# consensus-shipyard/ipc-filecoin-proofs

Hardware: NVIDIA H100
Metric: receipts/sec scanned (higher is better)
Workload: dtype u8

## Files before the change

ipc_filecoin_proofs_b200/csrc/engine.cuh:

```cuda
#pragma once
#include <array>
#include <memory>
#include <mutex>
#include <string>
#include <vector>

#include "common.cuh"
#include "store.cuh"
#include "rawcid.cuh"

namespace ipcfp {

struct NumaPrefer {
    bool on = false;
    int old_mode = 0;
    unsigned long old_mask[16] = {};
    explicit NumaPrefer(int device);
    ~NumaPrefer();
};

struct PinnedPool {
    struct Buf { void* p; size_t cap; };
    std::mutex mu;
    std::vector<Buf> free_list;
// ... 7 lines not shown
    size_t cap = 0;
    PinnedArray() {}
    PinnedArray(std::shared_ptr<PinnedPool> pl, size_t bytes) : pool(std::move(pl)) { p = pool->take(bytes ? bytes : 16, &cap); }
    PinnedArray(const PinnedArray&) = delete;
    PinnedArray& operator=(const PinnedArray&) = delete;
    PinnedArray(PinnedArray&& o) noexcept : pool(std::move(o.pool)), p(o.p), cap(o.cap) { o.p = nullptr; }
    PinnedArray& operator=(PinnedArray&& o) noexcept { release(); pool = std::move(o.pool); p = o.p; cap = o.cap; o.p = nullptr; return *this; }
    ~PinnedArray() { release(); }
    void release() { if (p && pool) pool->give(p, cap); p = nullptr; }
    template <class T> T* as() const { return (T*)p; }
};

struct Store {
    int device = 0;
    cudaStream_t stream = nullptr, stream2 = nullptr;
    uint64_t n = 0, blob_size = 0;
    DevBuf<uint8_t> arena;
    DevBuf<uint64_t> offsets;
    DevBuf<uint32_t> lengths;
    DevBuf<Digest> digests;
    DevBuf<uint8_t> cls;
    DevBuf<uint64_t> table;
    DevBuf<BlockRec> recs;
    DevBuf<uint32_t> rank_of, block_at_rank;
    StoreView view{};
    DevBuf<StoreView> view_dev;
    std::vector<std::array<uint8_t, 6>> class_prefix;
    std::vector<uint32_t> class_rank;
    uint64_t first_bad = UINT64_MAX;
    std::shared_ptr<PinnedPool> pool;
// ... 181 lines not shown
```

ipc_filecoin_proofs_b200/csrc/events.cu:

```cuda
#include <algorithm>
#include <cstdlib>
#include <cstring>

#include <chrono>
#include "engine.cuh"
#include "hashes.cuh"
#include "ipld.cuh"
#include "prims.cuh"
#include "walk.cuh"
#include "events_items.cuh"
#include "pass1_stage.cuh"
#include "rawcid.cuh"

namespace ipcfp {


__global__ void k_check_exec(const uint32_t* __restrict__ match_rel, uint64_t n_match, uint64_t lo, const unsigned long long* __restrict__ n_exec,
                             unsigned long long* err) {
    uint64_t t = (uint64_t)blockIdx.x * blockDim.x + threadIdx.x;
    if (t >= n_match) return;
    const uint64_t i = lo + match_rel[t];
    if (i >= *n_exec) report_error(err, ST_PASS2, i, 0 , 0);
}
__global__ void __launch_bounds__(128) k_pass2(Pass2Args a) {
    uint64_t t = (uint64_t)blockIdx.x * blockDim.x + threadIdx.x;
    if (a.per_warp) { if (threadIdx.x & 31) return; t >>= 5; }
    if (t >= a.n_match) return;
    pass2_item(a, t);
}

#define IPCFP_MAX_PARENTS 64
struct SetupArgs {
    StoreView store;
    uint32_t n_parents;
    const uint8_t* parent_cids;
    const uint8_t* txmeta_cids;
    const uint8_t* child_cid;
    const uint8_t* receipts_root;
    uint32_t skip_tx;
    uint32_t skip_receipts;
    uint32_t* wbits;
    unsigned long long* err;
    unsigned long long* txerr;
    uint32_t* receipts_root_blk;
    uint32_t* f_blk; uint32_t* f_meta; uint64_t* f_base;
    unsigned long long* f_count;
    uint32_t* amt_height;
    uint64_t* amt_count;
    uint32_t* missing_base;
    const uint8_t* sig;
    uint32_t sig_len;
    Matcher* matcher;
};

__global__ void __launch_bounds__(256) k_setup(SetupArgs a) {
    const StoreView& s = a.store;
    const uint32_t t = threadIdx.x, P = a.n_parents;
    if (t >= 128 && !a.skip_tx) {
        for (uint32_t i = t - 128; i < 2 * P + 2; i += 128) {
            const uint8_t* cid = i < P ? a.parent_cids + 38 * i : (i == P ? a.child_cid : (i == P + 1 ? a.receipts_root : a.txmeta_cids + 38 * (i - P - 2)));
            int32_t b = store_lookup(s, cid);
            if (b < 0) *a.missing_base = 1; else witness_mark(s, a.wbits, (uint32_t)b);
        }
    }
    if (t == 96) {
        Digest d;
        keccak256(a.sig, a.sig_len, d);
        a.matcher->t0[0] = d.w[0]; a.matcher->t0[1] = d.w[1]; a.matcher->t0[2] = d.w[2]; a.matcher->t0[3] = d.w[3];
    }
    if (t >= 32 && t < 96) for (uint32_t b = t - 32; b < P; b += 64) {
        for (uint32_t k = 0; k < 2; k++) { a.f_meta[2 * b + k] = AMT_SENTINEL; a.f_blk[2 * b + k] = 0; a.f_base[2 * b + k] = 0; a.amt_height[2 * b + k] = 0; a.amt_count[2 * b + k] = 0; }
        int32_t tb = store_lookup(s, a.txmeta_cids + 38 * b);
        if (tb < 0) { report_tx_error(a.txerr, 3 * b, 0, 31, DC_MISSING, 0); continue; }
        if (!a.skip_tx) witness_mark(s, a.wbits, (uint32_t)tb);
        uint32_t len;
        const uint8_t* p = store_block(s, (uint32_t)tb, len);
        Rd r(p, len);
        rd_array_exact(r, 2);
        uint32_t c0 = rd_cid(r), c1 = rd_cid(r);
        rd_end(r);
        if (r.err) { report_tx_error(a.txerr, 3 * b, 0, 31, DC_DECODE, r.err); continue; }
        for (uint32_t k = 0; k < 2; k++) {
            int32_t rb = store_lookup(s, p + (k ? c1 : c0));
            if (rb < 0) { report_tx_error(a.txerr, 3 * b + 1 + k, 0, 31, DC_MISSING, 0); break; }
            if (!a.skip_tx) witness_mark(s, a.wbits, (uint32_t)rb);
            uint32_t rl;
            const uint8_t* rp = store_block(s, (uint32_t)rb, rl);
            Rd rr(rp, rl);
            uint32_t bw, h;
            uint64_t cnt;
            amt_root_begin(rr, 0, bw, h, cnt);
            if (rr.err) { report_tx_error(a.txerr, 3 * b + 1 + k, 0, 31, DC_DECODE, rr.err); break; }
            const uint32_t amt = 2 * b + k;
            a.f_blk[amt] = (uint32_t)rb;
            a.f_meta[amt] = make_meta(amt, 1, h);
            a.f_base[amt] = 0;
            a.amt_height[amt] = h;
            a.amt_count[amt] = cnt;
        }
    }
    if (t != 0) return;
    *a.f_count = 2 * P;
    if (a.skip_receipts) return;
    int32_t rb = store_lookup(s, a.receipts_root);
    if (rb < 0) { report_error(a.err, ST_RECEIPTS_ROOT, 0, DC_MISSING, 0); return; }
    witness_mark(s, a.wbits, (uint32_t)rb);
    *a.receipts_root_blk = (uint32_t)rb;
    uint32_t len;
    const uint8_t* p = store_block(s, (uint32_t)rb, len);
    Rd r(p, len);
    uint32_t bw, h;
    uint64_t cnt;
    amt_root_begin(r, 0, bw, h, cnt);
    AmtNodeHdr hd;
    amt_node_begin(r, 3, hd);
    uint32_t nv = rd_array(r);
    for (uint32_t v = 0; v < nv && !r.err; v++) parse_receipt(r);
    amt_node_finish(r, hd, nv, h);
    if (r.err) report_error(a.err, ST_RECEIPTS_ROOT, 0, DC_DECODE, r.err);
}

__global__ void __launch_bounds__(128) k_amt_count(StoreView store, Frontier in, const unsigned long long* in_count, uint32_t round, uint32_t last_round,
                                                   uint32_t cap, uint32_t* counts, const uint64_t* rlo, const uint64_t* rhi) {
    uint64_t t = (uint64_t)blockIdx.x * blockDim.x + threadIdx.x;
    uint64_t cnt = *in_count;
    if (cnt > cap) cnt = cap;
    if (t >= cnt) { counts[t] = 0; return; }
    counts[t] = amt_item_count(store, in.blk[t], in.meta[t], in.base[t], round, last_round, rlo, rhi);
}
__global__ void __launch_bounds__(128) k_amt_expand(ExpandArgs a, const uint32_t* counts, unsigned long long* out_count, const unsigned long long* total) {
    const uint64_t g = (uint64_t)blockIdx.x * blockDim.x + threadIdx.x;
    const uint64_t t = g >> 3;
    const uint32_t j = (uint32_t)g & 7;
    uint64_t cnt = *a.in_count;
// ... 40 lines not shown
        ExpandArgs a = a0;
        a.in = cur; a.out = nxt; a.round = round; a.out_off = scan_tmp;
        for (uint32_t it = t >> 3; it < cnt; it += TOP_CAP / 8) amt_item_expand(a, it, t & 7, cur.blk[it], cur.meta[it], cur.base[it], s_cnt[it]);
        __syncthreads();
        if (t == 0) {
            unsigned long long n = s_total;
            if (round < a0.last_round && n > a0.cap) { report_tx_error(a0.err, IPCFP_TX_EIDX_NONE, 0, 0, DC_UNSUPPORTED, 1); n = a0.cap; }
            *count_io = n;
        }
        __threadfence();
        __syncthreads();
        Frontier tmp = cur; cur = nxt; nxt = tmp;
    }
}

__global__ void __launch_bounds__(1024) k_amt_dense(DenseArgs a, uint32_t first_round, uint32_t n_rounds) {
    for (uint32_t rr = 0; rr < n_rounds; rr++) {
        const uint32_t round = first_round + rr;
        if (*(volatile uint32_t*)a.fail) return;
        const Frontier in = (round & 1) ? a.pong : a.ping, out = (round & 1) ? a.ping : a.pong;
        const uint64_t n8 = (uint64_t)a.ftot[round] * 8;
        for (uint64_t g = (uint64_t)blockIdx.x * blockDim.x + threadIdx.x; g < n8; g += (uint64_t)gridDim.x * blockDim.x)
            amt_item_dense(a, in, out, round, (uint32_t)(g >> 3), (uint32_t)g & 7);
        if (n_rounds > 1) { __threadfence(); __syncthreads(); }
    }
}

__global__ void k_dedup_insert(const RawCid* __restrict__ raw, uint64_t n, unsigned long long* table, uint64_t mask) {
    uint64_t i = (uint64_t)blockIdx.x * blockDim.x + threadIdx.x;
    if (i >= n) return;
    RawCid c = raw[i];
    uint64_t h = rawcid_hash(c);
    uint32_t fp = (uint32_t)(h >> 32) | 1u;
    unsigned long long mine = ((unsigned long long)fp << 32) | (unsigned long long)(i + 1);
    uint64_t slot = h & mask;
    for (;;) {
        unsigned long long e = table[slot];
        if (e == 0) { e = atomicCAS(&table[slot], 0ull, mine); if (e == 0) return; }
        if ((uint32_t)(e >> 32) == fp && rawcid_eq(raw[(uint32_t)e - 1], c)) { atomicMin(&table[slot], mine); return; }
        slot = (slot + 1) & mask;
// ... 163 lines not shown
    {
        uint8_t* hs = s->stage.as<uint8_t>();
        memset(hs, 0, small_bytes);
        memcpy(hs, &mh, sizeof(Matcher));
        memcpy(hs + 1024, spec->event_signature, siglen);
        uint8_t* hc = hs + 1024 + sig_cap;
        memcpy(hc, td.parent_cids.data(), td.parent_cids.size()); hc += td.parent_cids.size();
        memcpy(hc, td.txmeta_cids.data(), td.txmeta_cids.size()); hc += td.txmeta_cids.size();
        memcpy(hc, td.child_cid, 38); hc += 38;
        memcpy(hc, td.receipts_root, 38);
        IPCFP_CUDA(cudaMemcpyAsync(small.p, hs, small_bytes, cudaMemcpyHostToDevice, st));
    }

    AsyncBuf<uint32_t> wbits((nblk + 31) / 32 + 8, st);
    wbits.zero();
    const uint32_t namt_max = 2 * td.n_parents;
    const uint64_t cap = 4 * nblk + 1024;
    AsyncBuf<uint32_t> fA_blk(cap, st), fA_meta(cap, st), fB_blk(cap, st), fB_meta(cap, st);
    AsyncBuf<uint64_t> fA_base(cap, st), fB_base(cap, st);
    AsyncBuf<uint32_t> misc(64 + 2 * IPCFP_MAX_PARENTS, st);
    AsyncBuf<uint64_t> amt_count(2 * IPCFP_MAX_PARENTS, st);
    misc.zero();
    SetupArgs sa;
    sa.store = s->view; sa.n_parents = td.n_parents;
    sa.parent_cids = d_cids; sa.txmeta_cids = d_cids + 38ull * td.n_parents;
    sa.child_cid = d_cids + 76ull * td.n_parents; sa.receipts_root = sa.child_cid + 38;
    sa.skip_tx = skip_tx; sa.skip_receipts = exo ? 1 : 0; sa.wbits = wbits.p; sa.err = dw; sa.txerr = dw + 15;
    sa.receipts_root_blk = misc.p; sa.missing_base = misc.p + 1; sa.amt_height = misc.p + 64;
    sa.f_blk = fA_blk.p; sa.f_meta = fA_meta.p; sa.f_base = fA_base.p; sa.f_count = dw + 1;
    sa.amt_count = amt_count.p;
    sa.sig = d_sig; sa.sig_len = (uint32_t)siglen; sa.matcher = d_matcher;
    k_setup<<<1, 256, 0, st>>>(sa); IPCFP_LAUNCH_CHECK();
    IPCFP_CUDA(cudaMemcpyAsync(hw + 400, d_matcher, 32, cudaMemcpyDeviceToHost, st));
    IPCFP_CUDA(cudaMemcpyAsync(hw + 24, misc.p, (64 + 2 * IPCFP_MAX_PARENTS) * 4, cudaMemcpyDeviceToHost, st));
    IPCFP_CUDA(cudaMemcpyAsync(hw + 128, amt_count.p, 2 * IPCFP_MAX_PARENTS * 8, cudaMemcpyDeviceToHost, st));
    IPCFP_CUDA(cudaMemcpyAsync(hw, dw, 16 * 8, cudaMemcpyDeviceToHost, st));
    IPCFP_CUDA(cudaStreamSynchronize(st));
    const bool early_fault = hw[0] != IPCFP_NO_ERROR || hw[15] != IPCFP_NO_ERROR;
    memcpy(mh.t0, hw + 400, 32);
    const uint32_t* misc_h = (const uint32_t*)(hw + 24);
    const uint32_t receipts_root_blk = misc_h[0];
    const bool missing_base = misc_h[1] != 0;
    uint32_t namt = (uint32_t)hw[1];
    uint32_t last_round = 0;
    for (uint32_t k = 0; k < namt && k < namt_max; k++) last_round = std::max(last_round, misc_h[64 + k]);

    IPCFP_CUDA(cudaEventRecord(s->ev[1], st));
    std::vector<uint64_t> h_rng(4 * IPCFP_MAX_PARENTS, 0);
    const uint64_t nraw_total = shard_amt_ranges(namt, (const uint64_t*)(hw + 128), sharded, lo, hi, td.n_receipts, h_rng.data(),
                                                 h_rng.data() + 2 * IPCFP_MAX_PARENTS);
    AsyncBuf<uint32_t> counts(cap + 1024, st);
    AsyncBuf<uint64_t> out_off(cap + 1024, st), scratch(scan_scratch_elems(std::max<uint64_t>(cap, N) + 64) + 64, st);
    unsigned long long *ccount = dw + 1, *ncount = dw + 2, *total_dev = dw + 13;
    const uint32_t frontier_cap = (uint32_t)std::min<uint64_t>(cap, 0xffffffffull);
    AsyncBuf<RawCid> exec_raw;
    uint64_t raw_cap = 0;

    const bool force_general = getenv("IPCFP_BFS_GENERAL") != nullptr;
    DensePlan plan;
    if (namt > 0 && namt <= namt_max && !force_general && !early_fault)
        plan = make_dense_plan(namt, misc_h + 64, (const uint64_t*)(hw + 128), h_rng.data(), h_rng.data() + 2 * IPCFP_MAX_PARENTS, frontier_cap, 8ull * cap,
                               STAGE_TABLES);
    AsyncBuf<uint8_t> d_tables;
    AsyncBuf<uint64_t> d_foff;
    AsyncBuf<uint32_t> d_flen;
    auto run_dense = [&]() {
        const size_t nb_amt = plan.per_amt.size() * 8, nb_fofs = plan.fofs.size() * 4, nb_ftot = plan.ftot.size() * 4;
        uint8_t* ht = s->stage.as<uint8_t>() + tables_off;
        memcpy(ht, plan.per_amt.data(), nb_amt);
        memcpy(ht + nb_amt, plan.fofs.data(), nb_fofs);
        memcpy(ht + nb_amt + nb_fofs, plan.ftot.data(), nb_ftot);
        d_tables.alloc(nb_amt + nb_fofs + nb_ftot + 64, st);
        IPCFP_CUDA(cudaMemcpyAsync(d_tables.p, ht, nb_amt + nb_fofs + nb_ftot, cudaMemcpyHostToDevice, st));
        raw_cap = plan.nraw;
        exec_raw.alloc(raw_cap + 64, st);
        exec_raw.zero();
        DenseArgs da;
        da.store = s->view;
        da.ping = Frontier{fA_blk.p, fA_meta.p, fA_base.p}; da.pong = Frontier{fB_blk.p, fB_meta.p, fB_base.p};
        da.vals = exec_raw.p;
        const uint64_t* pa = (const uint64_t*)d_tables.p;
        da.vbase = pa; da.cnt = pa + namt; da.lo = pa + 2ull * namt; da.hi = pa + 3ull * namt;
        da.fofs = (const uint32_t*)(d_tables.p + nb_amt); da.ftot = (const uint32_t*)(d_tables.p + nb_amt + nb_fofs);
        da.namt = namt; da.record = skip_tx ? 0 : 1; da.wbits = wbits.p; da.fail = (uint32_t*)(dw + 14);
        uint64_t fmax = 1;
        for (uint32_t r = 0; r < plan.rounds; r++) fmax = std::max<uint64_t>(fmax, plan.ftot[r]);
        d_foff.alloc(2 * fmax + 8, st); d_flen.alloc(2 * fmax + 8, st);
        da.f_off[0] = d_foff.p; da.f_off[1] = d_foff.p + fmax; da.f_len[0] = d_flen.p; da.f_len[1] = d_flen.p + fmax;
        uint32_t top = 0;
        while (top < plan.rounds && plan.ftot[top] <= 1024) top++;
        if (top) { k_amt_dense<<<1, 1024, 0, st>>>(da, 0, top); IPCFP_LAUNCH_CHECK(); }
        for (uint32_t r = top; r < plan.rounds; r++) {
            k_amt_dense<<<div_up((uint64_t)plan.ftot[r] * 8, 256), 256, 0, st>>>(da, r, 1); IPCFP_LAUNCH_CHECK();
        }
    };

    AsyncBuf<uint64_t> d_rng;
    auto run_general = [&]() {
        d_rng.alloc(4 * IPCFP_MAX_PARENTS, st);
        IPCFP_CUDA(cudaMemcpyAsync(d_rng.p, h_rng.data(), h_rng.size() * 8, cudaMemcpyHostToDevice, st));
        IPCFP_CUDA(cudaStreamSynchronize(st));
        Frontier fcur{fA_blk.p, fA_meta.p, fA_base.p}, fnxt{fB_blk.p, fB_meta.p, fB_base.p};
        ccount = dw + 1; ncount = dw + 2;
        ExpandArgs ea;
        ea.store = s->view; ea.last_round = last_round; ea.record = skip_tx ? 0 : 1; ea.wbits = wbits.p; ea.err = dw + 15;
        ea.vals = nullptr; ea.cap = frontier_cap;
        ea.rlo = d_rng.p; ea.rhi = d_rng.p + 2 * IPCFP_MAX_PARENTS;
        auto bound_of = [&](uint32_t round) { uint64_t b = namt; for (uint32_t k = 0; k < round && b <= cap; k++) b *= 8; return std::min<uint64_t>(b, cap); };
        auto alloc_vals = [&]() {
            raw_cap = std::min<uint64_t>(bound_of(last_round) * 8, 8 * cap);
// ... 13 lines not shown
            round = top_rounds;
        }
        for (; round <= last_round; round++) {
            uint64_t items = bound_of(round);
            if (round == last_round) alloc_vals();
            unsigned grid = div_up(std::max<uint64_t>(items, 1), 128);
            k_amt_count<<<grid, 128, 0, st>>>(s->view, fcur, ccount, round, last_round, ea.cap, counts.p, ea.rlo, ea.rhi); IPCFP_LAUNCH_CHECK();
            exclusive_scan_u32(counts.p, out_off.p, (uint64_t)grid * 128, (uint64_t*)total_dev, scratch.p, st);
            ExpandArgs a = ea;
            a.in = fcur; a.in_count = ccount; a.out = fnxt; a.round = round; a.out_off = out_off.p;
            k_amt_expand<<<div_up(std::max<uint64_t>(items, 1) * 8, 128), 128, 0, st>>>(a, counts.p, ncount, total_dev); IPCFP_LAUNCH_CHECK();
            std::swap(fcur, fnxt);
            std::swap(ccount, ncount);
        }
    };
    bool dense_used = plan.ok;
    if (dense_used) run_dense(); else run_general();
    IPCFP_CUDA(cudaEventRecord(s->ev[9], st));
    bool xch_early = false;
    if (xch) {
        xch->agree_early(plan.ok && !early_fault, plan.ok ? plan.nraw : 0, nraw_total);
        xch_early = xch->all_early;
        if (xch_early) xch->start_exchange(exec_raw.p, s->ev[9]);
    }
    WitnessBuilder wbuild(s);
    wbuild.by_ref = (flags & IPCFP_WITNESS_BY_REFERENCE) != 0;
    if (!exo) wbuild.snapshot(wbits.p);
    publish_words(s, 0, 18);
    IPCFP_CUDA(cudaStreamSynchronize(st));
    if (dense_used && hw[14] != 0) {
        dense_used = false;
        k_setup<<<1, 256, 0, st>>>(sa); IPCFP_LAUNCH_CHECK();
        run_general();
        IPCFP_CUDA(cudaEventRecord(s->ev[9], st));
        if (!exo) wbuild.snapshot(wbits.p);
        publish_words(s, 0, 18);
        IPCFP_CUDA(cudaStreamSynchronize(st));
    }
    const uint32_t ccount_idx = (uint32_t)(ccount - dw);
    note_errors(hw);
    if (!dense_used && hw[ccount_idx] > raw_cap) {
        if (!xch) throw Error(IPCFP_ERR_UNSUPPORTED, "unsupported input (message list longer than the walk's capacity)");
        pend_tx = std::min<uint64_t>(pend_tx, tx_err_key(IPCFP_TX_EIDX_NONE, 0, 0, DC_UNSUPPORTED, 1));
    }
    uint64_t nraw = dense_used ? plan.nraw : std::min<uint64_t>(hw[ccount_idx], raw_cap);
    bool xch_stale = xch_early && (!dense_used || nraw != plan.nraw);
    if (xch && !xch_early && (pend_tx != IPCFP_NO_ERROR || pend_err != IPCFP_NO_ERROR)) {
        xch->agree_slices(pend_tx, pend_err, 0);
        throw_global(xch->g_tx, xch->g_err, false);
    }
    if (!exo) wbuild.start_copy(hw[8], hw[9], hw[16], hw[17]);
    if (xch && !xch_early) {
        xch->agree_slices(IPCFP_NO_ERROR, IPCFP_NO_ERROR, nraw);
        if (!xch->peers_ok) { IPCFP_CUDA(cudaStreamSynchronize(st)); throw_global(xch->g_tx, xch->g_err, false); }
        xch->start_exchange(exec_raw.p, s->ev[9]);
    }
    AsyncBuf<uint32_t> exec_idx(nraw + 32, st), keep_bits((nraw + 31) / 32 + 8, st);
    unsigned long long* n_exec_dev = dw + 3;
    if (sharded) IPCFP_CUDA(cudaMemsetAsync(n_exec_dev, 0, 8, st));
    else if (nraw) {
// ... 34 lines not shown
    bitmap_to_indices(match_bits.p, (N + 31) / 32 * 32, match_rel.p, (uint64_t*)n_match_dev, wp3.p, scratch.p, st);
    exclusive_scan_u32(cnt.p, pbase.p, N, (uint64_t*)(dw + 7), scratch.p, st);
    exclusive_scan_u32(nby.p, bbase.p, N, (uint64_t*)(dw + 12), scratch.p, st);
    publish_words(s, 0, 16);
    IPCFP_CUDA(cudaStreamSynchronize(st));
    note_errors(hw);
    uint64_t n_exec = hw[3];
    const uint64_t M = hw[6];
    const uint64_t pass1_nodes = hw[4], pass1_bytes = hw[5];
    uint64_t n_proofs = hw[7], n_bytes = hw[12];

    std::unique_ptr<EventResultBox> box(new EventResultBox());
    memset(&box->r, 0, sizeof box->r);
    AsyncBuf<ipcfp_event_proof> d_proofs(n_proofs + 1, st);
    AsyncBuf<uint8_t> d_blob(n_bytes + 16, st);
    uint32_t* any_skip_dev = misc.p + 2;
    if (M) {
        Pass2Args p2;
        p2.store = s->view; p2.store_dev = s->view_dev.p; p2.m_dev = d_matcher; p2.m = mh; p2.events_roots = td.events_roots.p; p2.lo = lo; p2.match_rel = match_rel.p; p2.n_match = M;
        p2.receipts_root_blk = receipts_root_blk; p2.exec_cids = exec_raw.p; p2.exec_idx = exec_idx.p; p2.n_exec = n_exec_dev;
        p2.wbits = wbits.p; p2.err = dw; p2.cnt = cnt.p; p2.proof_base = pbase.p; p2.byte_base = bbase.p;
        p2.proofs = d_proofs.p; p2.blob = d_blob.p; p2.any_skip = any_skip_dev; p2.resolve_msg = sharded ? 0 : 1;
        p2.per_warp = (M <= 16384 && !getenv("IPCFP_PASS2_PER_THREAD")) ? 1 : 0;
        k_pass2<<<div_up(p2.per_warp ? M * 32 : M, 128), 128, 0, st>>>(p2); IPCFP_LAUNCH_CHECK();
    }
    if (xch) {
        cudaStream_t sx = xch->stream();
        xch->positions_for(sx, match_rel.p, M, n_exec_dev);
        IPCFP_CUDA(cudaMemsetAsync(dw + 19, 0xff, 8, sx));
        if (M) { k_check_exec<<<div_up(M, 128), 128, 0, sx>>>(match_rel.p, M, lo, n_exec_dev, dw + 19); IPCFP_LAUNCH_CHECK(); }
        publish_words_on(s, sx, dw + 19, 19, 1);
    }
    wbuild.finish_enqueue(wbits.p);
    publish_words(s, 0, 20);
    publish_words_from(s, misc.p, 20, 2);
    IPCFP_CUDA(cudaStreamSynchronize(st));
    note_errors(hw);
    if (!xch && missing_base && !skip_tx) throw Error(IPCFP_ERR_MISSING_BLOCK, "missing block (base witness CID not in the store)");
    const uint64_t mB = hw[10];
    const bool any_skip = ((const uint32_t*)(hw + 20))[2] != 0;
    IPCFP_CUDA(cudaEventRecord(s->ev[4], st));

    box->matching = PinnedArray(s->pool, (M + 1) * 8);
    box->proofs = PinnedArray(s->pool, (n_proofs + 1) * sizeof(ipcfp_event_proof));
    box->blob = PinnedArray(s->pool, n_bytes + 16);
    PinnedArray rel(s->pool, (M + 1) * 4);
    if (M) IPCFP_CUDA(cudaMemcpyAsync(rel.p, match_rel.p, M * 4, cudaMemcpyDeviceToHost, st));
    if (n_proofs && !xch) IPCFP_CUDA(cudaMemcpyAsync(box->proofs.p, d_proofs.p, n_proofs * sizeof(ipcfp_event_proof), cudaMemcpyDeviceToHost, st));
    if (n_bytes) IPCFP_CUDA(cudaMemcpyAsync(box->blob.p, d_blob.p, n_bytes, cudaMemcpyDeviceToHost, st));

// ... 137 lines not shown
```

ipc_filecoin_proofs_b200/csrc/walk.cuh:

```cuda
#pragma once
#include <algorithm>
#include <vector>

#include "ipld.cuh"
#include "rawcid.cuh"

namespace ipcfp {

__device__ __forceinline__ uint32_t make_meta(uint32_t amt, uint32_t is_root, uint32_t level) { return (amt << 16) | (is_root << 8) | level; }

#define AMT_SENTINEL 0xffffffffu

struct Frontier { uint32_t* blk; uint32_t* meta; uint64_t* base; };

__device__ __forceinline__ uint32_t slot_mask(uint64_t base, uint32_t level, uint64_t rlo, uint64_t rhi) {
    uint64_t sub = pow_sat(3, level);
    uint32_t m = 0;
#pragma unroll
    for (uint32_t sl = 0; sl < 8; sl++) {
        uint64_t off = sub == ~0ull ? (sl ? ~0ull : 0) : sub * sl;
        uint64_t cb = base + off < base ? ~0ull : base + off;
        uint64_t ce = cb + sub < cb ? ~0ull : cb + sub;
        if (cb < rhi && ce > rlo) m |= 1u << sl;
    }
// ... 79 lines not shown
                } else {
                    const uint8_t* src = p + vals_off + 43 * j + 5;
                    RawCid c;
                    c.w[4] = load_u64_any(src) & 0xffffffffffffull;
                    Digest dg = load_digest(src + 6);
                    c.w[0] = dg.w[0]; c.w[1] = dg.w[1]; c.w[2] = dg.w[2]; c.w[3] = dg.w[3];
                    a.vals[d] = c;
                }
            }
        }
    }
    if (a.round < a.last_round) for (uint32_t k = produced + j; k < expect; k += 8) if (o + k < a.cap) a.out.meta[o + k] = AMT_SENTINEL;
    if (a.round == a.last_round) for (uint32_t k = produced + j; k < expect; k += 8) { RawCid z{}; a.vals[o + k] = z; }
}

struct DenseArgs {
    StoreView store;
    Frontier ping, pong;
    RawCid* vals;
    const uint32_t* fofs;
    const uint32_t* ftot;
    const uint64_t* vbase;
    const uint64_t* cnt;
    const uint64_t* lo;
    const uint64_t* hi;
    uint32_t namt, record;
    uint32_t* wbits;
    uint32_t* fail;
    uint64_t* f_off[2];
    uint32_t* f_len[2];
};
__device__ __forceinline__ void amt_item_dense(const DenseArgs& a, const Frontier& in, const Frontier& out, uint32_t round, uint32_t it, uint32_t j) {
    const uint32_t meta = in.meta[it];
    const uint64_t base = in.base[it];
    const uint32_t level = meta & 0xff, is_root = (meta >> 8) & 1, amt = meta >> 16;
    uint32_t len;
    const uint8_t* p;
    if (round == 0) p = store_block(a.store, in.blk[it], len);
    else { const uint32_t par = round & 1; len = a.f_len[par][it]; p = a.store.blob + a.f_off[par][it]; }
    uint32_t q0 = 0;
    if (is_root) {
        Rd r(p, len);
        uint32_t bw, h; uint64_t c;
        amt_root_begin(r, 0, bw, h, c);
        if (r.err) { *a.fail = 1; return; }
// ... 50 lines not shown
        glo = n_receipts ? (uint64_t)((__uint128_t)nraw_total * lo / n_receipts) : 0;
        ghi = n_receipts ? (uint64_t)((__uint128_t)nraw_total * hi / n_receipts) : 0;
    }
    for (uint32_t k = 0; k < namt; k++) {
        uint64_t A0 = rawbase[k], A1 = rawbase[k + 1];
        uint64_t l = glo > A0 ? glo - A0 : 0, h = ghi > A0 ? ghi - A0 : 0;
        if (!sharded) { l = 0; h = UINT64_MAX; }
        else if (glo >= A1 && !(A1 == A0 && glo == A0)) { l = h = 0; }
        else if (ghi >= A1) h = UINT64_MAX;
        if (h < l) h = l;
        range_lo[k] = l; range_hi[k] = h;
    }
    return nraw_total;
}

struct DensePlan {
    bool ok = false;
    uint32_t rounds = 0;
    uint64_t nraw = 0;
    std::vector<uint32_t> fofs, ftot;
    std::vector<uint64_t> per_amt;
};
inline DensePlan make_dense_plan(uint32_t namt, const uint32_t* heights, const uint64_t* cnts, const uint64_t* range_lo, const uint64_t* range_hi,
                                 uint64_t frontier_cap, uint64_t max_raw, size_t max_table_bytes) {
    DensePlan plan;
    bool ok = namt > 0;
    uint32_t last_round = 0;
    for (uint32_t k = 0; ok && k < namt; k++) {
        ok = heights[k] <= 20 && cnts[k] <= (1ull << 40) && cnts[k] <= (1ull << (3 * (heights[k] + 1)));
        last_round = std::max(last_round, heights[k]);
    }
    if (ok) {
        plan.rounds = last_round + 1;
        plan.fofs.assign((size_t)plan.rounds * namt, 0);
        plan.ftot.assign(plan.rounds, 0);
        plan.per_amt.assign(4ull * namt, 0);
        uint64_t vb = 0;
        for (uint32_t k = 0; k < namt; k++) {
            const uint64_t c = cnts[k];
            const uint64_t l = std::min(range_lo[k], c), h = std::max(l, std::min(range_hi[k], c));
            if (l == h && l > 0) ok = false;
            plan.per_amt[k] = vb; plan.per_amt[namt + k] = c; plan.per_amt[2ull * namt + k] = l; plan.per_amt[3ull * namt + k] = h;
            vb += h - l;
        }
        plan.nraw = vb;
        for (uint32_t r = 0; ok && r < plan.rounds; r++) {
            uint64_t run = 0;
            for (uint32_t k = 0; k < namt; k++) {
                plan.fofs[(size_t)r * namt + k] = (uint32_t)run;
                const uint32_t hk = heights[k];
                if (r > hk) continue;
                const uint64_t l = plan.per_amt[2ull * namt + k], h = plan.per_amt[3ull * namt + k];
                const uint32_t sh = 3 * (hk - r + 1);
                uint64_t nodes = r == 0 ? 1 : (l < h ? (sh >= 64 ? 1 : ((h - 1) >> sh) - (l >> sh) + 1) : 0);
                run += nodes;
                if (run > frontier_cap) { ok = false; break; }
            }
            plan.ftot[r] = (uint32_t)run;
        }
        const size_t tbytes = plan.fofs.size() * 4 + plan.ftot.size() * 4 + plan.per_amt.size() * 8 + 64;
        if (plan.nraw > max_raw || tbytes > max_table_bytes) ok = false;
    }
    plan.ok = ok;
    return plan;
}

}
```

Measured before the change: 549.9 million.

## Build dense AMT walk plan on device and run walk as cooperative kernel

Moves the dense-walk planning from the host onto the device, inside the setup kernel, for the non-sharded case. This removes the mid-pipeline stream synchronize and device-to-host copy of the prologue that the host planner needed. The per-round walk launches are replaced by one cooperative kernel that uses grid.sync between levels, followed by a separate leaf kernel. The cost is a conservatively sized raw buffer (max_raw_dev), the exec_raw zeroing is dropped on the device-planned path, and the walk now depends on cooperative launch and grid occupancy.

```diff
diff --git a/ipc_filecoin_proofs_b200/csrc/engine.cuh b/ipc_filecoin_proofs_b200/csrc/engine.cuh
--- a/ipc_filecoin_proofs_b200/csrc/engine.cuh
+++ b/ipc_filecoin_proofs_b200/csrc/engine.cuh
@@ -45,6 +45,7 @@
 struct Store {
     int device = 0;
     cudaStream_t stream = nullptr, stream2 = nullptr;
+    unsigned walk_grid = 0;
     uint64_t n = 0, blob_size = 0;
     DevBuf<uint8_t> arena;
     DevBuf<uint64_t> offsets;
diff --git a/ipc_filecoin_proofs_b200/csrc/events.cu b/ipc_filecoin_proofs_b200/csrc/events.cu
--- a/ipc_filecoin_proofs_b200/csrc/events.cu
+++ b/ipc_filecoin_proofs_b200/csrc/events.cu
@@ -3,6 +3,8 @@
 #include <cstring>
 
 #include <chrono>
+#include <cstddef>
+#include <cooperative_groups.h>
 #include "engine.cuh"
 #include "hashes.cuh"
 #include "ipld.cuh"
@@ -13,6 +15,7 @@
 #include "rawcid.cuh"
 
 namespace ipcfp {
+namespace cg = cooperative_groups;
 
 
 __global__ void k_check_exec(const uint32_t* __restrict__ match_rel, uint64_t n_match, uint64_t lo, const unsigned long long* __restrict__ n_exec,
@@ -30,6 +33,16 @@
 }
 
 #define IPCFP_MAX_PARENTS 64
+static_assert(2 * IPCFP_MAX_PARENTS <= DENSE_MAX_AMTS, "the dense plan's tables hold every message AMT");
+struct Prologue {
+    uint32_t misc[64 + 2 * IPCFP_MAX_PARENTS];
+    uint64_t amt_count[2 * IPCFP_MAX_PARENTS];
+    uint64_t t0[4];
+    DenseTables plan;
+};
+#define PRO_HOST_WORD 24
+static constexpr uint32_t PRO_HEAD_WORDS = (uint32_t)((offsetof(Prologue, plan) + offsetof(DenseTables, per_amt)) / 8);
+static_assert(PRO_HOST_WORD + PRO_HEAD_WORDS <= 300, "the prologue's head must not reach the sharded protocol's host words");
 struct SetupArgs {
     StoreView store;
     uint32_t n_parents;
@@ -42,34 +55,55 @@
     uint32_t* wbits;
     unsigned long long* err;
     unsigned long long* txerr;
-    uint32_t* receipts_root_blk;
+    Prologue* pro;
     uint32_t* f_blk; uint32_t* f_meta; uint64_t* f_base;
     unsigned long long* f_count;
-    uint32_t* amt_height;
-    uint64_t* amt_count;
-    uint32_t* missing_base;
     const uint8_t* sig;
     uint32_t sig_len;
     Matcher* matcher;
+    uint32_t plan_dense;
+    uint64_t frontier_cap, max_raw;
 };
+
+__device__ __forceinline__ void setup_receipts_root(const SetupArgs& a) {
+    const StoreView& s = a.store;
+    int32_t rb = store_lookup(s, a.receipts_root);
+    if (rb < 0) { report_error(a.err, ST_RECEIPTS_ROOT, 0, DC_MISSING, 0); return; }
+    witness_mark(s, a.wbits, (uint32_t)rb);
+    a.pro->misc[0] = (uint32_t)rb;
+    uint32_t len;
+    const uint8_t* p = store_block(s, (uint32_t)rb, len);
+    Rd r(p, len);
+    uint32_t bw, h;
+    uint64_t cnt;
+    amt_root_begin(r, 0, bw, h, cnt);
+    AmtNodeHdr hd;
+    amt_node_begin(r, 3, hd);
+    uint32_t nv = rd_array(r);
+    for (uint32_t v = 0; v < nv && !r.err; v++) parse_receipt(r);
+    amt_node_finish(r, hd, nv, h);
+    if (r.err) report_error(a.err, ST_RECEIPTS_ROOT, 0, DC_DECODE, r.err);
+}
 
 __global__ void __launch_bounds__(256) k_setup(SetupArgs a) {
     const StoreView& s = a.store;
     const uint32_t t = threadIdx.x, P = a.n_parents;
+    uint32_t* const amt_height = a.pro->misc + 64;
+    uint64_t* const amt_count = a.pro->amt_count;
     if (t >= 128 && !a.skip_tx) {
         for (uint32_t i = t - 128; i < 2 * P + 2; i += 128) {
             const uint8_t* cid = i < P ? a.parent_cids + 38 * i : (i == P ? a.child_cid : (i == P + 1 ? a.receipts_root : a.txmeta_cids + 38 * (i - P - 2)));
             int32_t b = store_lookup(s, cid);
-            if (b < 0) *a.missing_base = 1; else witness_mark(s, a.wbits, (uint32_t)b);
+            if (b < 0) a.pro->misc[1] = 1; else witness_mark(s, a.wbits, (uint32_t)b);
         }
     }
     if (t == 96) {
         Digest d;
         keccak256(a.sig, a.sig_len, d);
-        a.matcher->t0[0] = d.w[0]; a.matcher->t0[1] = d.w[1]; a.matcher->t0[2] = d.w[2]; a.matcher->t0[3] = d.w[3];
+        for (int k = 0; k < 4; k++) a.matcher->t0[k] = a.pro->t0[k] = d.w[k];
     }
     if (t >= 32 && t < 96) for (uint32_t b = t - 32; b < P; b += 64) {
-        for (uint32_t k = 0; k < 2; k++) { a.f_meta[2 * b + k] = AMT_SENTINEL; a.f_blk[2 * b + k] = 0; a.f_base[2 * b + k] = 0; a.amt_height[2 * b + k] = 0; a.amt_count[2 * b + k] = 0; }
+        for (uint32_t k = 0; k < 2; k++) { a.f_meta[2 * b + k] = AMT_SENTINEL; a.f_blk[2 * b + k] = 0; a.f_base[2 * b + k] = 0; amt_height[2 * b + k] = 0; amt_count[2 * b + k] = 0; }
         int32_t tb = store_lookup(s, a.txmeta_cids + 38 * b);
         if (tb < 0) { report_tx_error(a.txerr, 3 * b, 0, 31, DC_MISSING, 0); continue; }
         if (!a.skip_tx) witness_mark(s, a.wbits, (uint32_t)tb);
@@ -95,29 +129,28 @@
             a.f_blk[amt] = (uint32_t)rb;
             a.f_meta[amt] = make_meta(amt, 1, h);
             a.f_base[amt] = 0;
-            a.amt_height[amt] = h;
-            a.amt_count[amt] = cnt;
-        }
-    }
+            amt_height[amt] = h;
+            amt_count[amt] = cnt;
+        }
+    }
+    if (t == 0) {
+        *a.f_count = 2 * P;
+        if (!a.skip_receipts) setup_receipts_root(a);
+    }
+    if (!a.plan_dense) return;
+    __syncthreads();
     if (t != 0) return;
-    *a.f_count = 2 * P;
-    if (a.skip_receipts) return;
-    int32_t rb = store_lookup(s, a.receipts_root);
-    if (rb < 0) { report_error(a.err, ST_RECEIPTS_ROOT, 0, DC_MISSING, 0); return; }
-    witness_mark(s, a.wbits, (uint32_t)rb);
-    *a.receipts_root_blk = (uint32_t)rb;
-    uint32_t len;
-    const uint8_t* p = store_block(s, (uint32_t)rb, len);
-    Rd r(p, len);
-    uint32_t bw, h;
-    uint64_t cnt;
-    amt_root_begin(r, 0, bw, h, cnt);
-    AmtNodeHdr hd;
-    amt_node_begin(r, 3, hd);
-    uint32_t nv = rd_array(r);
-    for (uint32_t v = 0; v < nv && !r.err; v++) parse_receipt(r);
-    amt_node_finish(r, hd, nv, h);
-    if (r.err) report_error(a.err, ST_RECEIPTS_ROOT, 0, DC_DECODE, r.err);
+    const uint32_t namt = 2 * P;
+    DenseTables& pl = a.pro->plan;
+    for (uint32_t k = 0; k < namt; k++) { pl.per_amt[2ull * namt + k] = 0; pl.per_amt[3ull * namt + k] = UINT64_MAX; }
+    uint32_t rounds;
+    uint64_t nraw;
+    const bool ok = dense_plan(namt, amt_height, amt_count, pl.per_amt + 2ull * namt, pl.per_amt + 3ull * namt, a.frontier_cap, a.max_raw, sizeof(DenseTables),
+                               pl.fofs, pl.ftot, pl.per_amt, &rounds, &nraw);
+    const bool fault = *(volatile unsigned long long*)a.err != IPCFP_NO_ERROR || *(volatile unsigned long long*)a.txerr != IPCFP_NO_ERROR;
+    pl.rounds = rounds;
+    pl.nraw = nraw;
+    pl.ok = ok && !fault;
 }
 
 __global__ void __launch_bounds__(128) k_amt_count(StoreView store, Frontier in, const unsigned long long* in_count, uint32_t round, uint32_t last_round,
@@ -188,16 +221,31 @@
     }
 }
 
-__global__ void __launch_bounds__(1024) k_amt_dense(DenseArgs a, uint32_t first_round, uint32_t n_rounds) {
-    for (uint32_t rr = 0; rr < n_rounds; rr++) {
-        const uint32_t round = first_round + rr;
-        if (*(volatile uint32_t*)a.fail) return;
-        const Frontier in = (round & 1) ? a.pong : a.ping, out = (round & 1) ? a.ping : a.pong;
-        const uint64_t n8 = (uint64_t)a.ftot[round] * 8;
-        for (uint64_t g = (uint64_t)blockIdx.x * blockDim.x + threadIdx.x; g < n8; g += (uint64_t)gridDim.x * blockDim.x)
-            amt_item_dense(a, in, out, round, (uint32_t)(g >> 3), (uint32_t)g & 7);
-        if (n_rounds > 1) { __threadfence(); __syncthreads(); }
-    }
+#define DENSE_THREADS 256
+__global__ void __launch_bounds__(DENSE_THREADS) k_amt_dense(DenseArgs a) {
+    const DenseTables& tb = *a.tables;
+    if (!tb.ok) { if (blockIdx.x == 0 && threadIdx.x == 0) *a.fail = 1; return; }
+    cg::grid_group grid = cg::this_grid();
+    const uint64_t stride = (uint64_t)gridDim.x * blockDim.x;
+    for (uint32_t round = 0; round + 1 < tb.rounds; round++) {
+        if (!*(volatile uint32_t*)a.fail) {
+            const Frontier in = (round & 1) ? a.pong : a.ping, out = (round & 1) ? a.ping : a.pong;
+            const uint64_t n8 = (uint64_t)tb.ftot[round] * 8;
+            for (uint64_t g = (uint64_t)blockIdx.x * blockDim.x + threadIdx.x; g < n8; g += stride)
+                amt_item_dense(a, in, out, round, (uint32_t)(g >> 3), (uint32_t)g & 7);
+        }
+        if (round + 2 < tb.rounds) grid.sync();
+    }
+}
+__global__ void __launch_bounds__(DENSE_THREADS) k_amt_dense_leaf(DenseArgs a) {
+    const DenseTables& tb = *a.tables;
+    if (!tb.ok) { if (blockIdx.x == 0 && threadIdx.x == 0) *a.fail = 1; return; }
+    if (*(volatile uint32_t*)a.fail) return;
+    const uint32_t round = tb.rounds - 1;
+    const Frontier in = (round & 1) ? a.pong : a.ping, out = (round & 1) ? a.ping : a.pong;
+    const uint64_t n8 = (uint64_t)tb.ftot[round] * 8;
+    for (uint64_t g = (uint64_t)blockIdx.x * blockDim.x + threadIdx.x; g < n8; g += (uint64_t)gridDim.x * blockDim.x)
+        amt_item_dense(a, in, out, round, (uint32_t)(g >> 3), (uint32_t)g & 7);
 }
 
 __global__ void k_dedup_insert(const RawCid* __restrict__ raw, uint64_t n, unsigned long long* table, uint64_t mask) {
@@ -391,86 +439,102 @@
 
     AsyncBuf<uint32_t> wbits((nblk + 31) / 32 + 8, st);
     wbits.zero();
-    const uint32_t namt_max = 2 * td.n_parents;
+    const uint32_t namt = 2 * td.n_parents;
     const uint64_t cap = 4 * nblk + 1024;
     AsyncBuf<uint32_t> fA_blk(cap, st), fA_meta(cap, st), fB_blk(cap, st), fB_meta(cap, st);
     AsyncBuf<uint64_t> fA_base(cap, st), fB_base(cap, st);
-    AsyncBuf<uint32_t> misc(64 + 2 * IPCFP_MAX_PARENTS, st);
-    AsyncBuf<uint64_t> amt_count(2 * IPCFP_MAX_PARENTS, st);
-    misc.zero();
+    AsyncBuf<Prologue> pro(1, st);
+    pro.zero();
+    uint32_t* const misc = &pro.p->misc[0];
+    const uint32_t frontier_cap = (uint32_t)std::min<uint64_t>(cap, 0xffffffffull);
+    const uint64_t max_raw_dev = std::min<uint64_t>(8ull * cap, (uint64_t)td.n_parents * td.n_receipts + 1024);
+    const bool force_general = getenv("IPCFP_BFS_GENERAL") != nullptr;
+    const bool plan_on_device = !sharded && !exo && !force_general;
     SetupArgs sa;
     sa.store = s->view; sa.n_parents = td.n_parents;
     sa.parent_cids = d_cids; sa.txmeta_cids = d_cids + 38ull * td.n_parents;
     sa.child_cid = d_cids + 76ull * td.n_parents; sa.receipts_root = sa.child_cid + 38;
     sa.skip_tx = skip_tx; sa.skip_receipts = exo ? 1 : 0; sa.wbits = wbits.p; sa.err = dw; sa.txerr = dw + 15;
-    sa.receipts_root_blk = misc.p; sa.missing_base = misc.p + 1; sa.amt_height = misc.p + 64;
+    sa.pro = pro.p;
     sa.f_blk = fA_blk.p; sa.f_meta = fA_meta.p; sa.f_base = fA_base.p; sa.f_count = dw + 1;
-    sa.amt_count = amt_count.p;
     sa.sig = d_sig; sa.sig_len = (uint32_t)siglen; sa.matcher = d_matcher;
+    sa.plan_dense = plan_on_device ? 1 : 0; sa.frontier_cap = frontier_cap; sa.max_raw = max_raw_dev;
     k_setup<<<1, 256, 0, st>>>(sa); IPCFP_LAUNCH_CHECK();
-    IPCFP_CUDA(cudaMemcpyAsync(hw + 400, d_matcher, 32, cudaMemcpyDeviceToHost, st));
-    IPCFP_CUDA(cudaMemcpyAsync(hw + 24, misc.p, (64 + 2 * IPCFP_MAX_PARENTS) * 4, cudaMemcpyDeviceToHost, st));
-    IPCFP_CUDA(cudaMemcpyAsync(hw + 128, amt_count.p, 2 * IPCFP_MAX_PARENTS * 8, cudaMemcpyDeviceToHost, st));
-    IPCFP_CUDA(cudaMemcpyAsync(hw, dw, 16 * 8, cudaMemcpyDeviceToHost, st));
-    IPCFP_CUDA(cudaStreamSynchronize(st));
-    const bool early_fault = hw[0] != IPCFP_NO_ERROR || hw[15] != IPCFP_NO_ERROR;
-    memcpy(mh.t0, hw + 400, 32);
-    const uint32_t* misc_h = (const uint32_t*)(hw + 24);
-    const uint32_t receipts_root_blk = misc_h[0];
-    const bool missing_base = misc_h[1] != 0;
-    uint32_t namt = (uint32_t)hw[1];
-    uint32_t last_round = 0;
-    for (uint32_t k = 0; k < namt && k < namt_max; k++) last_round = std::max(last_round, misc_h[64 + k]);
-
     IPCFP_CUDA(cudaEventRecord(s->ev[1], st));
+
+    const Prologue* ph = (const Prologue*)(hw + PRO_HOST_WORD);
+    auto publish_prologue = [&]() { publish_words_from(s, pro.p, PRO_HOST_WORD, PRO_HEAD_WORDS); };
+    bool early_fault = false, missing_base = false;
+    uint32_t receipts_root_blk = 0, last_round = 0;
     std::vector<uint64_t> h_rng(4 * IPCFP_MAX_PARENTS, 0);
-    const uint64_t nraw_total = shard_amt_ranges(namt, (const uint64_t*)(hw + 128), sharded, lo, hi, td.n_receipts, h_rng.data(),
-                                                 h_rng.data() + 2 * IPCFP_MAX_PARENTS);
+    uint64_t nraw_total = 0;
+    auto read_prologue = [&]() {
+        early_fault = hw[0] != IPCFP_NO_ERROR || hw[15] != IPCFP_NO_ERROR;
+        memcpy(mh.t0, ph->t0, 32);
+        receipts_root_blk = ph->misc[0];
+        missing_base = ph->misc[1] != 0;
+        last_round = 0;
+        for (uint32_t k = 0; k < namt; k++) last_round = std::max(last_round, ph->misc[64 + k]);
+        nraw_total = shard_amt_ranges(namt, ph->amt_count, sharded, lo, hi, td.n_receipts, h_rng.data(), h_rng.data() + 2 * IPCFP_MAX_PARENTS);
+    };
+
     AsyncBuf<uint32_t> counts(cap + 1024, st);
     AsyncBuf<uint64_t> out_off(cap + 1024, st), scratch(scan_scratch_elems(std::max<uint64_t>(cap, N) + 64) + 64, st);
     unsigned long long *ccount = dw + 1, *ncount = dw + 2, *total_dev = dw + 13;
-    const uint32_t frontier_cap = (uint32_t)std::min<uint64_t>(cap, 0xffffffffull);
     AsyncBuf<RawCid> exec_raw;
     uint64_t raw_cap = 0;
 
-    const bool force_general = getenv("IPCFP_BFS_GENERAL") != nullptr;
     DensePlan plan;
-    if (namt > 0 && namt <= namt_max && !force_general && !early_fault)
-        plan = make_dense_plan(namt, misc_h + 64, (const uint64_t*)(hw + 128), h_rng.data(), h_rng.data() + 2 * IPCFP_MAX_PARENTS, frontier_cap, 8ull * cap,
-                               STAGE_TABLES);
-    AsyncBuf<uint8_t> d_tables;
+    if (!plan_on_device) {
+        publish_words(s, 0, 16);
+        publish_prologue();
+        IPCFP_CUDA(cudaStreamSynchronize(st));
+        read_prologue();
+        if (namt > 0 && !force_general && !early_fault)
+            plan = make_dense_plan(namt, ph->misc + 64, ph->amt_count, h_rng.data(), h_rng.data() + 2 * IPCFP_MAX_PARENTS, frontier_cap, 8ull * cap,
+                                   sizeof(DenseTables));
+    }
     AsyncBuf<uint64_t> d_foff;
     AsyncBuf<uint32_t> d_flen;
+    DenseArgs da;
+    memset(&da, 0, sizeof da);
     auto run_dense = [&]() {
-        const size_t nb_amt = plan.per_amt.size() * 8, nb_fofs = plan.fofs.size() * 4, nb_ftot = plan.ftot.size() * 4;
-        uint8_t* ht = s->stage.as<uint8_t>() + tables_off;
-        memcpy(ht, plan.per_amt.data(), nb_amt);
-        memcpy(ht + nb_amt, plan.fofs.data(), nb_fofs);
-        memcpy(ht + nb_amt + nb_fofs, plan.ftot.data(), nb_ftot);
-        d_tables.alloc(nb_amt + nb_fofs + nb_ftot + 64, st);
-        IPCFP_CUDA(cudaMemcpyAsync(d_tables.p, ht, nb_amt + nb_fofs + nb_ftot, cudaMemcpyHostToDevice, st));
-        raw_cap = plan.nraw;
+        if (!plan_on_device) {
+            static_assert(sizeof(DenseTables) <= STAGE_TABLES, "the dense plan must fit its staging slot");
+            DenseTables* ht = (DenseTables*)(s->stage.as<uint8_t>() + tables_off);
+            memset(ht, 0, sizeof *ht);
+            ht->ok = 1; ht->rounds = plan.rounds; ht->nraw = plan.nraw;
+            std::copy(plan.per_amt.begin(), plan.per_amt.end(), ht->per_amt);
+            std::copy(plan.fofs.begin(), plan.fofs.end(), ht->fofs);
+            std::copy(plan.ftot.begin(), plan.ftot.end(), ht->ftot);
+            IPCFP_CUDA(cudaMemcpyAsync(&pro.p->plan, ht, sizeof(DenseTables), cudaMemcpyHostToDevice, st));
+        }
+        raw_cap = plan_on_device ? max_raw_dev : plan.nraw;
         exec_raw.alloc(raw_cap + 64, st);
-        exec_raw.zero();
-        DenseArgs da;
+        if (!plan_on_device) exec_raw.zero();
+        const DenseTables* tb = &pro.p->plan;
         da.store = s->view;
         da.ping = Frontier{fA_blk.p, fA_meta.p, fA_base.p}; da.pong = Frontier{fB_blk.p, fB_meta.p, fB_base.p};
         da.vals = exec_raw.p;
-        const uint64_t* pa = (const uint64_t*)d_tables.p;
-        da.vbase = pa; da.cnt = pa + namt; da.lo = pa + 2ull * namt; da.hi = pa + 3ull * namt;
-        da.fofs = (const uint32_t*)(d_tables.p + nb_amt); da.ftot = (const uint32_t*)(d_tables.p + nb_amt + nb_fofs);
+        da.tables = tb;
+        da.vbase = tb->per_amt; da.cnt = tb->per_amt + namt; da.lo = tb->per_amt + 2ull * namt; da.hi = tb->per_amt + 3ull * namt;
+        da.fofs = tb->fofs; da.ftot = tb->ftot;
         da.namt = namt; da.record = skip_tx ? 0 : 1; da.wbits = wbits.p; da.fail = (uint32_t*)(dw + 14);
         uint64_t fmax = 1;
-        for (uint32_t r = 0; r < plan.rounds; r++) fmax = std::max<uint64_t>(fmax, plan.ftot[r]);
+        if (plan_on_device) fmax = max_raw_dev / 8 + namt + 8;
+        else for (uint32_t r = 0; r < plan.rounds; r++) fmax = std::max<uint64_t>(fmax, plan.ftot[r]);
         d_foff.alloc(2 * fmax + 8, st); d_flen.alloc(2 * fmax + 8, st);
         da.f_off[0] = d_foff.p; da.f_off[1] = d_foff.p + fmax; da.f_len[0] = d_flen.p; da.f_len[1] = d_flen.p + fmax;
-        uint32_t top = 0;
-        while (top < plan.rounds && plan.ftot[top] <= 1024) top++;
-        if (top) { k_amt_dense<<<1, 1024, 0, st>>>(da, 0, top); IPCFP_LAUNCH_CHECK(); }
-        for (uint32_t r = top; r < plan.rounds; r++) {
-            k_amt_dense<<<div_up((uint64_t)plan.ftot[r] * 8, 256), 256, 0, st>>>(da, r, 1); IPCFP_LAUNCH_CHECK();
-        }
+        if (!s->walk_grid) {
+            int per_sm = 0, sms = 0;
+            IPCFP_CUDA(cudaOccupancyMaxActiveBlocksPerMultiprocessor(&per_sm, k_amt_dense, DENSE_THREADS, 0));
+            IPCFP_CUDA(cudaDeviceGetAttribute(&sms, cudaDevAttrMultiProcessorCount, s->device));
+            s->walk_grid = (unsigned)std::max(1, per_sm * sms);
+        }
+        void* args[] = {&da};
+        IPCFP_CUDA(cudaLaunchCooperativeKernel((const void*)k_amt_dense, s->walk_grid, DENSE_THREADS, args, 0, st)); IPCFP_LAUNCH_CHECK();
     };
+    auto run_dense_leaf = [&]() { k_amt_dense_leaf<<<s->walk_grid, DENSE_THREADS, 0, st>>>(da); IPCFP_LAUNCH_CHECK(); };
 
     AsyncBuf<uint64_t> d_rng;
     auto run_general = [&]() {
@@ -514,8 +578,8 @@
             std::swap(ccount, ncount);
         }
     };
-    bool dense_used = plan.ok;
-    if (dense_used) run_dense(); else run_general();
+    bool dense_used = plan_on_device || plan.ok;
+    if (dense_used) { run_dense(); run_dense_leaf(); } else run_general();
     IPCFP_CUDA(cudaEventRecord(s->ev[9], st));
     bool xch_early = false;
     if (xch) {
@@ -527,7 +591,9 @@
     wbuild.by_ref = (flags & IPCFP_WITNESS_BY_REFERENCE) != 0;
     if (!exo) wbuild.snapshot(wbits.p);
     publish_words(s, 0, 18);
+    if (plan_on_device) publish_prologue();
     IPCFP_CUDA(cudaStreamSynchronize(st));
+    if (plan_on_device) read_prologue();
     if (dense_used && hw[14] != 0) {
         dense_used = false;
         k_setup<<<1, 256, 0, st>>>(sa); IPCFP_LAUNCH_CHECK();
@@ -543,7 +609,7 @@
         if (!xch) throw Error(IPCFP_ERR_UNSUPPORTED, "unsupported input (message list longer than the walk's capacity)");
         pend_tx = std::min<uint64_t>(pend_tx, tx_err_key(IPCFP_TX_EIDX_NONE, 0, 0, DC_UNSUPPORTED, 1));
     }
-    uint64_t nraw = dense_used ? plan.nraw : std::min<uint64_t>(hw[ccount_idx], raw_cap);
+    uint64_t nraw = dense_used ? (plan_on_device ? ph->plan.nraw : plan.nraw) : std::min<uint64_t>(hw[ccount_idx], raw_cap);
     bool xch_stale = xch_early && (!dense_used || nraw != plan.nraw);
     if (xch && !xch_early && (pend_tx != IPCFP_NO_ERROR || pend_err != IPCFP_NO_ERROR)) {
         xch->agree_slices(pend_tx, pend_err, 0);
@@ -608,7 +674,7 @@
     memset(&box->r, 0, sizeof box->r);
     AsyncBuf<ipcfp_event_proof> d_proofs(n_proofs + 1, st);
     AsyncBuf<uint8_t> d_blob(n_bytes + 16, st);
-    uint32_t* any_skip_dev = misc.p + 2;
+    uint32_t* any_skip_dev = misc + 2;
     if (M) {
         Pass2Args p2;
         p2.store = s->view; p2.store_dev = s->view_dev.p; p2.m_dev = d_matcher; p2.m = mh; p2.events_roots = td.events_roots.p; p2.lo = lo; p2.match_rel = match_rel.p; p2.n_match = M;
@@ -627,7 +693,7 @@
     }
     wbuild.finish_enqueue(wbits.p);
     publish_words(s, 0, 20);
-    publish_words_from(s, misc.p, 20, 2);
+    publish_words_from(s, misc, 20, 2);
     IPCFP_CUDA(cudaStreamSynchronize(st));
     note_errors(hw);
     if (!xch && missing_base && !skip_tx) throw Error(IPCFP_ERR_MISSING_BLOCK, "missing block (base witness CID not in the store)");
diff --git a/ipc_filecoin_proofs_b200/csrc/walk.cuh b/ipc_filecoin_proofs_b200/csrc/walk.cuh
--- a/ipc_filecoin_proofs_b200/csrc/walk.cuh
+++ b/ipc_filecoin_proofs_b200/csrc/walk.cuh
@@ -117,6 +117,7 @@
     if (a.round == a.last_round) for (uint32_t k = produced + j; k < expect; k += 8) { RawCid z{}; a.vals[o + k] = z; }
 }
 
+struct DenseTables;
 struct DenseArgs {
     StoreView store;
     Frontier ping, pong;
@@ -132,6 +133,7 @@
     uint32_t* fail;
     uint64_t* f_off[2];
     uint32_t* f_len[2];
+    const DenseTables* tables;
 };
 __device__ __forceinline__ void amt_item_dense(const DenseArgs& a, const Frontier& in, const Frontier& out, uint32_t round, uint32_t it, uint32_t j) {
     const uint32_t meta = in.meta[it];
@@ -212,6 +214,57 @@
     return nraw_total;
 }
 
+#define DENSE_MAX_AMTS 128
+#define DENSE_MAX_ROUNDS 21
+__host__ __device__ inline bool dense_plan(uint32_t namt, const uint32_t* heights, const uint64_t* cnts, const uint64_t* range_lo, const uint64_t* range_hi,
+                                           uint64_t frontier_cap, uint64_t max_raw, size_t max_table_bytes, uint32_t* fofs, uint32_t* ftot,
+                                           uint64_t* per_amt, uint32_t* rounds_out, uint64_t* nraw_out) {
+    *rounds_out = 0; *nraw_out = 0;
+    bool ok = namt > 0 && namt <= DENSE_MAX_AMTS;
+    uint32_t last_round = 0;
+    for (uint32_t k = 0; ok && k < namt; k++) {
+        ok = heights[k] <= 20 && cnts[k] <= (1ull << 40) && cnts[k] <= (1ull << (3 * (heights[k] + 1)));
+        last_round = heights[k] > last_round ? heights[k] : last_round;
+    }
+    if (!ok) return false;
+    const uint32_t rounds = last_round + 1;
+    uint64_t vb = 0;
+    for (uint32_t k = 0; k < namt; k++) {
+        const uint64_t c = cnts[k];
+        const uint64_t l = range_lo[k] < c ? range_lo[k] : c;
+        const uint64_t hc = range_hi[k] < c ? range_hi[k] : c, h = hc > l ? hc : l;
+        if (l == h && l > 0) ok = false;
+        per_amt[k] = vb; per_amt[namt + k] = c; per_amt[2ull * namt + k] = l; per_amt[3ull * namt + k] = h;
+        vb += h - l;
+    }
+    for (uint32_t r = 0; ok && r < rounds; r++) {
+        uint64_t run = 0;
+        for (uint32_t k = 0; k < namt; k++) {
+            fofs[(size_t)r * namt + k] = (uint32_t)run;
+            const uint32_t hk = heights[k];
+            if (r > hk) continue;
+            const uint64_t l = per_amt[2ull * namt + k], h = per_amt[3ull * namt + k];
+            const uint32_t sh = 3 * (hk - r + 1);
+            uint64_t nodes = r == 0 ? 1 : (l < h ? (sh >= 64 ? 1 : ((h - 1) >> sh) - (l >> sh) + 1) : 0);
+            run += nodes;
+            if (run > frontier_cap) { ok = false; break; }
+        }
+        ftot[r] = (uint32_t)run;
+    }
+    const size_t tbytes = (size_t)rounds * namt * 4 + (size_t)rounds * 4 + 4ull * namt * 8 + 64;
+    if (vb > max_raw || tbytes > max_table_bytes) ok = false;
+    *rounds_out = rounds; *nraw_out = vb;
+    return ok;
+}
+
+struct DenseTables {
+    uint32_t ok, rounds;
+    uint64_t nraw;
+    uint64_t per_amt[4 * DENSE_MAX_AMTS];
+    uint32_t fofs[DENSE_MAX_ROUNDS * DENSE_MAX_AMTS];
+    uint32_t ftot[DENSE_MAX_ROUNDS];
+};
+
 struct DensePlan {
     bool ok = false;
     uint32_t rounds = 0;
@@ -222,44 +275,13 @@
 inline DensePlan make_dense_plan(uint32_t namt, const uint32_t* heights, const uint64_t* cnts, const uint64_t* range_lo, const uint64_t* range_hi,
                                  uint64_t frontier_cap, uint64_t max_raw, size_t max_table_bytes) {
     DensePlan plan;
-    bool ok = namt > 0;
-    uint32_t last_round = 0;
-    for (uint32_t k = 0; ok && k < namt; k++) {
-        ok = heights[k] <= 20 && cnts[k] <= (1ull << 40) && cnts[k] <= (1ull << (3 * (heights[k] + 1)));
-        last_round = std::max(last_round, heights[k]);
-    }
-    if (ok) {
-        plan.rounds = last_round + 1;
-        plan.fofs.assign((size_t)plan.rounds * namt, 0);
-        plan.ftot.assign(plan.rounds, 0);
-        plan.per_amt.assign(4ull * namt, 0);
-        uint64_t vb = 0;
-        for (uint32_t k = 0; k < namt; k++) {
-            const uint64_t c = cnts[k];
-            const uint64_t l = std::min(range_lo[k], c), h = std::max(l, std::min(range_hi[k], c));
-            if (l == h && l > 0) ok = false;
-            plan.per_amt[k] = vb; plan.per_amt[namt + k] = c; plan.per_amt[2ull * namt + k] = l; plan.per_amt[3ull * namt + k] = h;
-            vb += h - l;
-        }
-        plan.nraw = vb;
-        for (uint32_t r = 0; ok && r < plan.rounds; r++) {
-            uint64_t run = 0;
-            for (uint32_t k = 0; k < namt; k++) {
-                plan.fofs[(size_t)r * namt + k] = (uint32_t)run;
-                const uint32_t hk = heights[k];
-                if (r > hk) continue;
-                const uint64_t l = plan.per_amt[2ull * namt + k], h = plan.per_amt[3ull * namt + k];
-                const uint32_t sh = 3 * (hk - r + 1);
-                uint64_t nodes = r == 0 ? 1 : (l < h ? (sh >= 64 ? 1 : ((h - 1) >> sh) - (l >> sh) + 1) : 0);
-                run += nodes;
-                if (run > frontier_cap) { ok = false; break; }
-            }
-            plan.ftot[r] = (uint32_t)run;
-        }
-        const size_t tbytes = plan.fofs.size() * 4 + plan.ftot.size() * 4 + plan.per_amt.size() * 8 + 64;
-        if (plan.nraw > max_raw || tbytes > max_table_bytes) ok = false;
-    }
-    plan.ok = ok;
+    plan.fofs.assign((size_t)DENSE_MAX_ROUNDS * namt, 0);
+    plan.ftot.assign(DENSE_MAX_ROUNDS, 0);
+    plan.per_amt.assign(4ull * namt, 0);
+    plan.ok = dense_plan(namt, heights, cnts, range_lo, range_hi, frontier_cap, max_raw, max_table_bytes, plan.fofs.data(), plan.ftot.data(),
+                         plan.per_amt.data(), &plan.rounds, &plan.nraw);
+    plan.fofs.resize((size_t)plan.rounds * namt);
+    plan.ftot.resize(plan.rounds);
     return plan;
 }
 
```

New measurement: 599.2 million (median of 6 runs). 1.09x the previous value.
